# tyler-a-cox/fftvis

Hardware: AMD Instinct MI355X
Metric: simulated visibilities/sec (baselines x freqs x times) at eps=6e-8 (higher is better)
Workload: dtype f64; 1 GPU; C3: hera350, 100000 sources, 128 freqs, 20 times, 61075 baselines, polarized table beam, type3 NUFFT eps=6e-08 upsampfac=2

## Files before the change

### fftvis_amd/csrc/fv_nufft.h

```cpp
#pragma once

#include "fv_eskernel.h"
#include "fv_ydirect.h"

#include <hip/hip_ext.h>

#include <algorithm>
#include <cstdlib>
#include <array>
#include <map>
#include <memory>

namespace fv {

inline bool debug_switch_old_fft() {
    static const bool v = std::getenv("FFTVIS_HIP_OLD_FFT") != nullptr;
    return v;
}
inline bool debug_switch_natural_order() {
    static const bool v = std::getenv("FFTVIS_HIP_NATURAL_ORDER") != nullptr;
    return v;
}

constexpr int BINLOG = 3;
// ... 2701 lines not shown
            DimGeom g;
            g.X = X[d];
            g.B = B[d];
            set_dim_geom(g, sigma, ker.w, scale_max, true, 0.0);
            cells *= g.n2;
        }
        return cells >= 4.0e6 ? -1.0 : 0.0;
    }
    int *col_err = nullptr;
    const unsigned long long *col_omask = nullptr;
    int col_omask_nblk = 0;
    double col_out_cells = 0;
    void arm_columns(const int *tab, const int *xtab, int tpol, int ncc, int *err = nullptr, const unsigned long long *omask = nullptr,
                     int omask_nblk = 0) {
        col_tab = tab && xtab && (dim == 2 || zdirect) && b_block_log() ? tab : nullptr;
        col_xtab = col_tab ? xtab : nullptr;
        col_tab_tpol = tpol;
        col_ncc = ncc;
        col_err = err;
        col_omask = col_tab ? omask : nullptr;
        col_omask_nblk = omask_nblk;
        col_out_cells = 0;
    }
    bool yd_on = false;
    YdArgs yd_args{};
    const int *yd_map = nullptr;
    double yd_cells = 0, yd_pairs = 0;
    DevBuf yd_vals, yd_ones;
    int yd_ones_n = 0;
    const double *yd_scale = nullptr;
    void arm_ydirect(const YdArgs *a, const int *map, double b_cells, const double *scale_dev = nullptr) {
        yd_on = a != nullptr && sizeof(T) == 8 && dim == 2;
        if (!yd_on) return;
        yd_args = *a;
        yd_map = map;
        yd_scale = scale_dev;
        yd_cells = b_cells;
        yd_pairs = (double)a->npts * geo.d[1].na;
    }
    int yd_slots = 0;
    int yd_slot_count() {
        if (!yd_slots) {
            const int smem = (int)yd_smem_bytes();
            int dev = 0, cus = 0, per_cu = 0;
            FV_HIP(hipFuncSetAttribute(reinterpret_cast<const void *>(k_ydirect), hipFuncAttributeMaxDynamicSharedMemorySize, smem));
            FV_HIP(hipOccupancyMaxActiveBlocksPerMultiprocessor(&per_cu, k_ydirect, YD_THREADS, (size_t)smem));
            FV_HIP(hipGetDevice(&dev));
            FV_HIP(hipDeviceGetAttribute(&cus, hipDeviceAttributeMultiprocessorCount, dev));
            yd_slots = std::max(1, per_cu * cus);
        }
        return yd_slots;
    }
    static constexpr int YD_MAX_SLICES = 32;
    void yd_slices(int na_y, int nwg, int nft, int &rps, int &nslices) {
        const int tiles = (int)cdiv(na_y, YD_RT);
        const char *e = std::getenv("FFTVIS_HIP_YD_SLICES");
        int want = e ? std::atoi(e) : 0;
        if (want < 1) {
            const int64_t slots = yd_slot_count(), base = (int64_t)std::max(1, nwg) * std::max(1, nft);
            int64_t best = 0;
            for (int n = 1; n <= std::min(tiles, YD_MAX_SLICES); ++n) {
                const int tps = (int)cdiv(tiles, n), ns = (int)cdiv(tiles, tps);
                const int64_t cost = (2 * cdiv(base * ns, slots) + 1) * (tps + 1);
                if (!want || cost < best) {
                    best = cost;
                    want = n;
                }
            }
        }
        want = std::max(1, std::min(want, tiles));
        rps = (int)cdiv(tiles, want) * YD_RT;
        nslices = (int)cdiv(na_y, rps);
    }
    size_t yd_vals_bytes(int na_y, int nwg, int nfg, int tg, int64_t npts) {
        int rps, ns;
        yd_slices(na_y, nwg, nfg * tg, rps, ns);
        return sizeof(cplx<double>) * (size_t)ns * nfg * tg * (size_t)npts;
    }
    const T *spread_dec_y() {
        if (!yd_on) return dec_cur[1];
        const int n = geo.d[1].na;
        if (yd_ones_n < n) {
            if (yd_ones.p) FV_HIP(hipStreamSynchronize(stream));
            const int cap = std::max(n, 16384);
            yd_ones.reserve(sizeof(double) * (size_t)cap);
            hipLaunchKernelGGL(k_yd_ones, dim3((unsigned)cdiv(cap, 256)), dim3(256), 0, stream, yd_ones.as<double>(), cap);
            yd_ones_n = cap;
        }
        return reinterpret_cast<const T *>(yd_ones.p);
    }
    void ydirect_sum(int ntrans, const cplx<T> *B);
    int ypass_cols_log() const {
        int tpr, rpw;
        rowfft_shape(geo.d[1], true, tpr, rpw);
        return ilog2_c(rpw);
    }
    void build_rowmask(int64_t NU, const T *btx, const T *bty, const int *bl_idx, const signed char *flip, const int *ustart,
                       const double *scale_dev, int nfg, bool both, const int *ctab, int ncc, unsigned long long *mask,
                       int nblk, int nw) const {
        const DimGeom &x = geo.d[0], &y = geo.d[1];
        RowMaskArgs a{};
        a.w = ker.w;
        a.nfg = nfg;
        a.sides = both ? 2 : 1;
        a.n2x = x.n2; a.nox = x.no; a.Px = x.sP(); a.cntx = x.cnt(); a.hx = x.h; a.btcx = x.btc;
        a.n2y = y.n2; a.noy = y.no; a.Py = y.P; a.Qy = y.Q; a.hy = y.h; a.btcy = y.btc;
        a.blk_log = ypass_cols_log();
        a.nblk = nblk;
        a.nw = nw;
        a.ctab_stride = x.nos();
        (void)ncc;
        const int64_t items = NU * nfg * a.sides;
        if (items == 0) return;
        hipLaunchKernelGGL(k_plan_rowmask<T>, dim3((unsigned)cdiv(items, 256)), dim3(256), 0, stream, NU, btx, bty, bl_idx,
                           flip, ustart, scale_dev, a, ctab, mask);
    }
    int xcols() const { return col_tab ? col_ncc : geo.d[0].nos(); }
    int b_block_log_public() const { return b_block_log(); }
    int xcols_with(int ncc) const { return ncc ? ncc : geo.d[0].nos(); }
    int64_t b_pitch_with(int ncc) const { return y_reads_columns() ? (xcols_with(ncc) + 7) / 8 * 8 : xcols_with(ncc); }
    bool columns_possible() const { return (dim == 2 || zdirect) && b_block_log() != 0 && y_reads_columns() && !fused_possible(); }
    bool fused_possible() const;
    bool prepare_fused_gather(int64_t N, const T *btx, const T *bty, const int *bl_idx, const signed char *flip,
                              const double *scale_dev, int nfg, int tpol, cplx<T> *out, int64_t out_fg_stride,
                              int64_t out_k_stride, const int64_t *out_pol_off, int64_t targets_serial = 0,
                              cplx<T> *out_mate = nullptr);
    int64_t M = 0;
    int64_t geom_serial = 0;

// ... 681 lines not shown
    first_pass_ext = row_ext_ptr;
    rowfft(cur, oth, x, tw_cur[0], np, y.na, (int64_t)y.na * x.na, x.na, 1, xp, 0, nullptr, cur1, oth1, 0, blk);
    first_pass_ext = nullptr;
    std::swap(cur, oth);
    std::swap(cur1, oth1);
    if (yd_on) {
        FV_REQUIRE(!mate && !fused_active && dim == 2, "direct y sums: 2-D, stand-alone gather, no gang launch");
        ydirect_sum(ntrans, cur);
        grid_out = cur;
        last_fft_fused = false;
        return;
    }
    if (y_reads_columns()) {
        rowfft(cur, oth, y, tw_cur[1], np, xp, (int64_t)y.na * xp, 1, xp, 0, xcols(),
               fused_active ? &fused_args : nullptr, cur1, oth1, blk, 0);
        std::swap(cur, oth);
        std::swap(cur1, oth1);
    } else {
        dim3 tg((unsigned)cdiv(x.nos(), 32), (unsigned)cdiv(y.na, 32), (unsigned)np);
        hipLaunchKernelGGL(k_transpose<T>, tg, dim3(256), 0, stream, cur, oth, y.na, x.nos());
        if (mate) hipLaunchKernelGGL(k_transpose<T>, tg, dim3(256), 0, stream, cur1, oth1, y.na, x.nos());
        rowfft(oth, cur, y, tw_cur[1], np, x.nos(), (int64_t)x.nos() * y.na, y.na, 1, 0, 0, nullptr,
               oth1, cur1);
    }
    if (dim > 2 && !zdirect) {
        const int64_t nc = (int64_t)x.nos() * y.nos();
        rowfft(cur, oth, z, tw_cur[2], ntrans, nc, (int64_t)z.na * nc, 1, nc);
        std::swap(cur, oth);
    }
    grid_out = cur;
    last_fft_fused = fused_active;
    if (mate) {
        mate->grid_out = cur1;
        mate->last_fft_fused = fused_active;
    }
    fused_active = false;
}

template <typename T>
void Nufft3<T>::ydirect_sum(int ntrans, const cplx<T> *B) {
    if constexpr (sizeof(T) == 8) {
        const DimGeom &y = geo.d[1];
        YdArgs a = yd_args;
        const int tg = ntrans / std::max(1, a.nfg);
        FV_REQUIRE(a.nfg >= 1 && tg * a.nfg == ntrans && (tg == 1 || tg == 2 || tg == 4), "direct y sums: 1, 2 or 4 transforms per frequency");
        const int blk = b_block_log();
        FV_REQUIRE(a.na_y == y.na && a.xp == (int)b_pitch() && a.blk == (blk ? blk : 2) && a.w == ker.w,
                   "direct y sums: the tables were built for another geometry");
        a.plane = (int64_t)y.na * b_pitch();
        a.blk_stride = blk ? ((int64_t)y.na << blk) : 4;
        a.row_stride = blk ? (1 << blk) : b_pitch();
        a.tg = tg;
        FV_REQUIRE(a.blk >= 2 && a.blk <= 4 && a.plane < ((int64_t)1 << 31), "direct y sums: blocks of 4 to 16 elements, 32-bit cell offsets");
        yd_slices(y.na, a.nwg, ntrans, a.rps, a.nslices);
        const size_t need = sizeof(cplx<double>) * (size_t)a.nslices * ntrans * (size_t)a.npts;
        if (yd_vals.cap < need) {
            FV_HIP(hipStreamSynchronize(stream));
            yd_vals.reserve(need);
        }
        yd_args.rps = a.rps;
        yd_args.nslices = a.nslices;
        yd_slot_count();
        const dim3 grid((unsigned)a.nwg, (unsigned)ntrans, (unsigned)a.nslices);
        hipLaunchKernelGGL(k_ydirect, grid, dim3(YD_THREADS), yd_smem_bytes(), stream, reinterpret_cast<const cplx<double> *>(B),
                           yd_scale, a, yd_vals.as<cplx<double>>());
    } else {
        (void)ntrans;
        (void)B;
        FV_REQUIRE(false, "direct y sums: fp64 only");
    }
}

template <typename T>
bool Nufft3<T>::fused_possible() const {
    static const bool off = std::getenv("FFTVIS_HIP_NO_FUSED_GATHER") != nullptr;
    if (off || dim != 2) return false;
    const DimGeom &x = geo.d[0], &y = geo.d[1];
    int tpr, rpw;
    rowfft_shape(y, true, tpr, rpw);
    if (!rowfft_uses_st(y, true) || rpw != 8 || y.logQ > 10) return false;
    if (x.sP() != 1 || y.P != 1) return false;
    const int row_slots = y.logQ == 9 ? 577 : 1153;
    return 2 * y.no <= row_slots && b_pitch() % 8 == 0;
}

template <typename T>
bool Nufft3<T>::prepare_fused_gather(int64_t N, const T *btx, const T *bty, const int *bl_idx,
                                     const signed char *flip, const double *scale_dev, int nfg, int tpol,
                                     cplx<T> *out, int64_t out_fg_stride, int64_t out_k_stride,
                                     const int64_t *out_pol_off, int64_t targets_serial, cplx<T> *out_mate) {
    if (N == 0 || nfg == 0 || tpol > 4 || !fused_possible()) return false;
    const DimGeom &x = geo.d[0], &y = geo.d[1];
    FusedKey key;
    key.serial = geom_serial;
    key.targets = targets_serial;
    key.N = N;
    key.ofs = out_fg_stride;
    key.oks = out_k_stride;
    key.btx = btx;
    key.bl_idx = bl_idx;
    key.flip = flip;
    key.scale = scale_dev;
    key.nfg = nfg;
    key.tpol = tpol;
    const double kg[10] = {x.h, y.h, x.btc, y.btc, x.xc, y.xc, (double)x.no, (double)y.no, (double)x.n2, (double)y.n2};
    for (int i = 0; i < 10; ++i) key.g[i] = kg[i];
    FgGeom gm{};
// ... 240 lines not shown
```

### fftvis_amd/csrc/fv_sim.h

```cpp
#pragma once

#include <atomic>
#include <chrono>
#include <cstdio>
#include <thread>
#include "fv_fit.h"
#include "fv_nufft.h"
#include <unordered_map>

#include <algorithm>
#include <array>
#include <cstdlib>
#include <memory>

namespace fv {

constexpr double SPEED_OF_LIGHT = 299792458.0;

struct BeamDesc {
    int kind;
    int order;
    double diameter;
    double js[8];
    double ps;
// ... 2392 lines not shown
                        hi = std::min(x.no - 1, hi + 1);
                    }
                    for (int i = lo; i <= hi; ++i) row[out_pos(i, P, cnt)] = 1;
                }
            }
            int run = 0;
            for (int i = 0; i < stride; ++i)
                if (row[i]) row[i] = ++run;
            c->ncc = std::max(c->ncc, run);
            if (run * 100 > x.no * 85) c->use = false;
        }
        c->ncc = (c->ncc + 7) / 8 * 8;
        c->yn2 = y.n2; c->yno = y.no; c->yP = y.P; c->yQ = y.Q; c->yh = y.h; c->ybtc = y.btc;
        c->yna = y.na;
        c->blk = n0->b_block_log_public();
        if (c->use) {
            upload(c->tab, tab.data(), sizeof(int) * tab.size(), 0);
            c->h_tab = tab;
            {
                std::vector<int> xt(tab.size());
                const int b = c->blk, rows = y.na << b, mask = (1 << b) - 1;
                for (size_t i = 0; i < tab.size(); ++i) xt[i] = tab[i] ? ((tab[i] - 1) >> b) * rows + ((tab[i] - 1) & mask) + 1 : 0;
                upload(c->xtab, xt.data(), sizeof(int) * xt.size(), 0);
            }
            if (y.logQ >= 9 && y.logQ <= 11 && !std::getenv("FFTVIS_HIP_NO_OUTPUT_MASK")) {
                const int bl = n0->ypass_cols_log(), nw = y.Q > 1024 ? y.Q / 1024 : 1;
                c->nblk = (c->ncc + (1 << bl) - 1) >> bl;
                const size_t words = (size_t)nfg * c->nblk * y.P * nw;
                c->omask.reserve(sizeof(unsigned long long) * words);
                FV_HIP(hipMemsetAsync(c->omask.p, 0, sizeof(unsigned long long) * words, stream));
                hipStream_t keep = n0->stream;
                n0->stream = stream;
                n0->build_rowmask(nu, d_bls.as<T>(), d_bls.as<T>() + nbls, pr.trivial ? nullptr : pr.idx->template as<int>(),
                                  pr.trivial ? nullptr : pr.flip->template as<signed char>(),
                                  pr.ustart ? pr.ustart->template as<int>() : nullptr, d_freqs.as<double>() + fa, nfg, both,
                                  c->tab.template as<int>(), c->ncc, c->omask.template as<unsigned long long>(), c->nblk, nw);
                n0->stream = keep;
                std::vector<unsigned long long> hm(words);
                FV_HIP(hipMemcpyAsync(hm.data(), c->omask.p, sizeof(unsigned long long) * words, hipMemcpyDeviceToHost, stream));
                FV_HIP(hipStreamSynchronize(stream));
                double bits = 0;
                for (unsigned long long v : hm) bits += __builtin_popcountll(v);
                c->out_cells = bits * 16.0 * (1 << bl) / nfg;
            }
        }
        col_plans.push_back(std::move(c));
        return col_plans.back().get();
    }

    struct YPlan {
        int64_t serial;
        int pair, fa, fb;
        const ColPlan *cp;
        int herm, blk, xp, w;
        int xn2, xno, xsP, xcnt, yna, yn2;
        double xh, xbtc, yh, ybtc;
        bool built = false, use = false;
        YdArgs a{};
        double cells = 0;
        DevBuf wg, blkcnt, blkid, cref, xw, ptv, ptg, map;
    };
    std::vector<std::unique_ptr<YPlan>> y_plans;
    std::vector<YPlan *> y_plan_of;
    static double ydirect_gate() { return 1.0; }
    YPlan *ydirect_plan(int pi, const Pair &pr, int fa, int fb, Nufft3<T> *n0, const ColPlan *cp, bool forced) {
        const DimGeom &x = n0->geo.d[0], &y = n0->geo.d[1];
        const int w = n0->ker.w, blkB = n0->b_block_log_public(), blk = blkB ? blkB : 2;
        const int xp = (int)n0->b_pitch_with(cp && cp->use ? cp->ncc : 0);
        for (auto &c : y_plans)
            if (c->serial == targets_serial && c->pair == pi && c->fa == fa && c->fb == fb && c->cp == cp && c->herm == pr.herm &&
                c->blk == (blkB ? blkB : -2) && c->xp == xp && c->w == w && c->xn2 == x.n2 && c->xno == x.no && c->xsP == x.sP() &&
                c->xcnt == x.cnt() && c->yna == y.na && c->yn2 == y.n2 && c->xh == x.h && c->xbtc == x.btc && c->yh == y.h &&
                c->ybtc == y.btc)
                return c.get();
        std::unique_ptr<YPlan> c(new YPlan{targets_serial, pi, fa, fb, cp, pr.herm, blkB ? blkB : -2, xp, w, x.n2, x.no, x.sP(), x.cnt(),
                                           y.na, y.n2, x.h, x.btc, y.h, y.btc});
        y_plans.push_back(std::move(c));
        YPlan *yp = y_plans.back().get();
        const bool dbg = std::getenv("FFTVIS_HIP_DEBUG_YDIRECT") != nullptr;
        auto skip = [&](const char *why) {
            if (dbg) std::fprintf(stderr, "ydirect plan pair %d channels [%d, %d): not built: %s\n", pi, fa, fb, why);
            return yp;
        };
        const int nfg = fb - fa, BE = 1 << blk, sides = pr.herm ? 2 : 1;
        const int64_t N = !pr.h_upairs.empty() ? (int64_t)pr.h_upairs.size() / 2 : !pr.h_ustart.empty() ? (int64_t)pr.h_ustart.size() - 1 : pr.n;
        if (N == 0 || nfg == 0 || w > MAX_W || (pr.herm && (x.btc != 0.0 || y.btc != 0.0))) return skip("no items, or a packed run off centre");
        const size_t NP = (size_t)N * sides;
        std::vector<double> pu(NP), pv(NP);
        for (int64_t i = 0; i < N; ++i) {
            const int64_t ui = !pr.h_upairs.empty() ? pr.h_upairs[2 * i] : i;
            const int64_t kl = pr.h_ustart.empty() ? ui : pr.h_ustart[ui];
            const int64_t k = pr.h_idx[kl];
            const double sg = pr.h_flip[kl] ? -1.0 : 1.0;
            for (int sd = 0; sd < sides; ++sd) {
                const double s2 = sd ? -sg : sg;
                pu[(size_t)i * sides + sd] = s2 * (double)(T)h_bls[k];
                pv[(size_t)i * sides + sd] = s2 * (double)(T)h_bls[(size_t)nbls + k];
            }
        }
        const double tol = std::max(dedup_tol(), 0.0);
        std::vector<int> ord(NP), grp(NP), map(2 * (size_t)N, 0);
        for (size_t i = 0; i < NP; ++i) ord[i] = (int)i;
        std::sort(ord.begin(), ord.end(), [&](int p, int q) { return pu[p] < pu[q] || (pu[p] == pu[q] && (pv[p] < pv[q] || (pv[p] == pv[q] && p < q))); });
        std::vector<double> gu;
        for (size_t i = 0; i < NP; ++i) {
            if (gu.empty() || pu[ord[i]] - gu.back() > tol) gu.push_back(pu[ord[i]]);
            grp[ord[i]] = (int)gu.size() - 1;
        }
        const int G = (int)gu.size();
        std::sort(ord.begin(), ord.end(), [&](int p, int q) { return grp[p] < grp[q] || (grp[p] == grp[q] && (pv[p] < pv[q] || (pv[p] == pv[q] && p < q))); });
        std::vector<double> ptv;
        std::vector<int> ptg, gstart(G + 1, 0);
        for (size_t i = 0; i < NP; ++i) {
            const int q = ord[i];
            if (ptv.empty() || ptg.back() != grp[q] || pv[q] - ptv.back() > tol) {
                ptv.push_back(pv[q]);
                ptg.push_back(grp[q]);
                ++gstart[grp[q] + 1];
            }
            map[(size_t)(q / sides) * 2 + (q % sides)] = (int)ptv.size() - 1;
        }
        for (int g = 0; g < G; ++g) gstart[g + 1] += gstart[g];
        const int64_t npts = (int64_t)ptv.size();
        if (!forced && (double)npts * y.na > ydirect_gate() * ((double)G * w) * 0.5 * y.n2 * std::log2((double)y.n2)) return skip("too many points per u");
        if (blk < 2 || blk > 4) return skip("column blocks of fewer than 4 or more than 16 elements");
        if ((int64_t)y.na * xp >= ((int64_t)1 << 31)) return skip("a plane of B past the kernel's 32-bit cell offsets");
        const int P = x.sP(), cnt = x.cnt(), stride = x.nos(), ncols = n0->xcols_with(cp && cp->use ? cp->ncc : 0);
        const double beta = n0->ker.beta, c4 = n0->ker.c;
        std::vector<int> col((size_t)nfg * G * w);
        std::vector<double> xw((size_t)nfg * G * w);
        for (int fg = 0; fg < nfg; ++fg) {
            const double sc = freqs[fa + fg];
            for (int g = 0; g < G; ++g) {
                const double sv = sc * gu[g], th = x.h * (sv - sc * x.btc);
                const double e = th * x.n2 * (0.5 / M_PI) + 0.5 * x.no;
                const int j = std::max(0, std::min(x.no - w, (int)std::ceil(e - 0.5 * w)));
                for (int q = 0; q < w; ++q) {
                    const int pos = out_pos(std::min(j + q, x.no - 1), P, cnt);
                    int cc = pos;
                    if (cp && cp->use) {
                        const int t = cp->h_tab[(size_t)fg * stride + pos];
                        if (t == 0) return skip("a footprint column the column plan left out");
                        cc = t - 1;
                    }
                    if (cc < 0 || cc >= ncols || cc >= xp) return skip("a column outside B");
                    col[((size_t)fg * G + g) * w + q] = cc;
                    xw[((size_t)fg * G + g) * w + q] = es_eval<double>((double)(j + q) - e, beta, c4);
                }
            }
        }
        const int nbcap = yd_nbcap(blk);
        std::vector<int> wg;
        std::vector<std::vector<int>> cur(nfg), trial(nfg);
        auto blocks_with = [&](int g) {
            int worst = 0;
            for (int fg = 0; fg < nfg; ++fg) {
                trial[fg] = cur[fg];
                for (int q = 0; q < w; ++q) trial[fg].push_back(col[((size_t)fg * G + g) * w + q] >> blk);
                std::sort(trial[fg].begin(), trial[fg].end());
                trial[fg].erase(std::unique(trial[fg].begin(), trial[fg].end()), trial[fg].end());
                worst = std::max(worst, (int)trial[fg].size());
            }
            return worst;
        };
        std::vector<std::vector<int>> range_blocks;
        int g0 = 0;
        while (g0 < G) {
            for (auto &v : cur) v.clear();
            int ng = 0;
            while (g0 + ng < G && ng < YD_NG && gstart[g0 + ng + 1] - gstart[g0] <= YD_THREADS * YD_PTM) {
                if (blocks_with(g0 + ng) > nbcap) break;
                cur.swap(trial);
                ++ng;
            }
            if (ng == 0) return skip("one u-group alone does not fit a workgroup");
            wg.insert(wg.end(), {g0, ng, gstart[g0], gstart[g0 + ng] - gstart[g0]});
            for (int fg = 0; fg < nfg; ++fg) range_blocks.push_back(cur[fg]);
            g0 += ng;
        }
        const int nwg = (int)wg.size() / 4;
        std::vector<int> blkcnt((size_t)nfg * nwg), blkid((size_t)nfg * nwg * YD_NBMAX, 0), cref(col.size());
        double cells = 0;
        for (int r = 0; r < nwg; ++r)
            for (int fg = 0; fg < nfg; ++fg) {
                const std::vector<int> &bl = range_blocks[(size_t)r * nfg + fg];
                blkcnt[(size_t)fg * nwg + r] = (int)bl.size();
                cells += (double)bl.size() * BE * y.na / nfg;
                for (size_t i = 0; i < bl.size(); ++i) blkid[((size_t)fg * nwg + r) * YD_NBMAX + i] = bl[i];
                for (int g = wg[4 * r]; g < wg[4 * r] + wg[4 * r + 1]; ++g)
                    for (int q = 0; q < w; ++q) {
                        const int cc = col[((size_t)fg * G + g) * w + q];
                        const int slot = (int)(std::lower_bound(bl.begin(), bl.end(), cc >> blk) - bl.begin());
                        cref[((size_t)fg * G + g) * w + q] = (slot << 4) | (cc & (BE - 1));
                    }
            }
        upload(yp->wg, wg.data(), sizeof(int) * wg.size(), 0);
        upload(yp->blkcnt, blkcnt.data(), sizeof(int) * blkcnt.size(), 0);
        upload(yp->blkid, blkid.data(), sizeof(int) * blkid.size(), 0);
        upload(yp->cref, cref.data(), sizeof(int) * cref.size(), 0);
        upload(yp->xw, xw.data(), sizeof(double) * xw.size(), 0);
        upload(yp->ptv, ptv.data(), sizeof(double) * ptv.size(), 0);
        upload(yp->ptg, ptg.data(), sizeof(int) * ptg.size(), 0);
        upload(yp->map, map.data(), sizeof(int) * map.size(), 0);
        YdArgs &a = yp->a;
        a.w = w;
        a.nfg = nfg;
        a.nwg = nwg;
        a.ngroups = G;
        a.na_y = y.na;
        a.xp = xp;
        a.blk = blk;
        a.npts = npts;
        a.hy = y.h;
        a.btcy = y.btc;
        a.wg = yp->wg.template as<int>();
        a.blkcnt = yp->blkcnt.template as<int>();
        a.blkid = yp->blkid.template as<int>();
        a.cref = yp->cref.template as<int>();
        a.xw = yp->xw.template as<double>();
        a.ptv = yp->ptv.template as<double>();
        a.ptg = yp->ptg.template as<int>();
        yp->cells = cells;
        yp->built = true;
        std::vector<int> dc(col.begin() + (size_t)(nfg - 1) * G * w, col.end());
        std::sort(dc.begin(), dc.end());
        const double columns = (double)(std::unique(dc.begin(), dc.end()) - dc.begin());
        const double direct = (double)npts * y.na, ypass = columns * 0.5 * y.n2 * std::log2((double)y.n2);
        yp->use = n0->columns_possible() && n0->geo.cells_o() >= 4000000 && direct <= ydirect_gate() * ypass;
        if (dbg)
            std::fprintf(stderr, "ydirect plan pair %d channels [%d, %d): %lld items, %lld points on %d u-groups, %d work ranges, %.0f columns, "
                         "B cells read %.3g of %.3g needed, na_y %d, blocks of %d, plan %d, rule %.2f -> %s\n", pi, fa, fb, (long long)N,
                         (long long)npts, G, nwg, columns, cells, columns * y.na, y.na, BE, cp ? 1 : 0, direct / ypass, yp->use ? "taken" : "not taken");
        return yp;
    }

    void set_basis(int nant, int K, int nfreq, const void *coefs, const int *ant1,
                   const int *ant2) override {
        FV_HIP(hipSetDevice(device));
        FV_REQUIRE(polarized, "basis beams need a polarized engine (wrapper.py:280-283)");
        FV_REQUIRE(nbls > 0 && K >= 1 && K == (int)beams.size(), "set_array and the K basis beams first");
        FV_REQUIRE(nfreq == (int)freqs.size(), "beam_coefs frequency axis != freqs");
        for (int64_t b = 0; b < nbls; ++b)
            FV_REQUIRE(ant1[b] >= 0 && ant1[b] < nant && ant2[b] >= 0 && ant2[b] < nant, "antenna index out of range");
        nbasis = K;
        nant_basis = nant;
        {
            std::vector<int> start(nant + 1, 0), list((size_t)2 * nbls);
            for (int64_t b = 0; b < nbls; ++b) {
                ++start[ant1[b] + 1];
                ++start[ant2[b] + 1];
            }
            for (int a = 0; a < nant; ++a) start[a + 1] += start[a];
            std::vector<int> fill(start.begin(), start.end() - 1);
            for (int64_t b = 0; b < nbls; ++b) {
                list[fill[ant1[b]]++] = (int)(2 * b);
                list[fill[ant2[b]]++] = (int)(2 * b + 1);
            }
            upload(d_csr_start, start.data(), sizeof(int) * start.size(), 0);
            upload(d_csr, list.data(), sizeof(int) * list.size(), 0);
        }
        upload(d_coefs, coefs, sizeof(cplx<T>) * (size_t)nant * K * nfreq, 0);
        upload(d_ant1, ant1, sizeof(int) * nbls, 0);
        upload(d_ant2, ant2, sizeof(int) * nbls, 0);
        std::vector<int> bi, bj, idx(nbls);
        std::vector<int64_t> off(1, 0);
        std::vector<int> all;
        std::vector<signed char> fl;
        for (int k = 0; k < K; ++k)
            for (int l = k; l < K; ++l) {
                bi.push_back(k);
                bj.push_back(l);
                for (int64_t b = 0; b < nbls; ++b) {
                    all.push_back((int)b);
                    fl.push_back(0);
                }
                off.push_back((int64_t)all.size());
            }
        set_beam_pairs((int)bi.size(), bi.data(), bj.data(), off.data(), all.data(), fl.data());
    }

    void set_chunking(int nchunks, double sb) override {
        FV_REQUIRE(nchunks >= 1, "nchunks must be >= 1");
        FV_REQUIRE(sb > 0.0 && sb <= 1.0, "source_buffer must be in (0, 1]");
        src_chunks = nchunks;
        source_buffer = sb;
// ... 893 lines not shown
        }
        for (auto &cpo : col_plan_of) cpo.assign(r.groups.size() * pairs.size(), nullptr);
        if (col_plans.size() > 512) {
            FV_HIP(hipDeviceSynchronize());
            col_plans.clear();
            y_plans.clear();
        }
        if (y_plans.size() > 512) {
            FV_HIP(hipDeviceSynchronize());
            y_plans.clear();
        }
        y_plan_of.assign(r.groups.size() * pairs.size(), nullptr);
        for (int c = 0; c < r.ncls; ++c) {
            if (std::getenv("FFTVIS_HIP_NO_COLUMN_PLAN")) break;
            Nufft3<T> *n0 = lanes[0].plan[c].get();
            if (n0->dim != 2 && !n0->zdirect) continue;
            for (size_t gi = 0; gi < r.groups.size(); ++gi) {
                const double smax = fmax_of(r.groups[gi].first, r.groups[gi].second);
                for (size_t pi = 0; pi < pairs.size(); ++pi) {
                    const Pair &pr = pairs[pi];
                    if (pr.n == 0) continue;
                    n0->grid_slack = 0.0;
                    n0->set_geometry(r.xc, r.X, pr.box_c(), pr.box_B(), smax);
                    if (!n0->columns_possible() || n0->geo.cells_o() < 4000000) continue;
                    col_plan_of[c][gi * pairs.size() + pi] = column_plan((int)pi, pr, r.groups[gi].first, r.groups[gi].second, n0);
                }
            }
            FV_HIP(hipStreamSynchronize(n0->stream));
        }
        const char *ey = std::getenv("FFTVIS_HIP_YDIRECT");
        const int ymode = ey ? std::atoi(ey) : -1;
        if (!r.forward || ymode == 0 || sizeof(T) != 8 || r.D != 2 || r.gang || nbasis || r.K || r.nsets()) return;
        Nufft3<T> *n0 = lanes[0].plan[0].get();
        size_t vals_need = 0;
        for (size_t gi = 0; gi < r.groups.size(); ++gi) {
            const int fa = r.groups[gi].first, fb = r.groups[gi].second;
            const double smax = fmax_of(fa, fb);
            for (size_t pi = 0; pi < pairs.size(); ++pi) {
                const Pair &pr = pairs[pi];
                const int tg = pr.herm ? 2 : tpol;
                if (pr.n == 0 || tg > 4 || pr.mirror) continue;
                const ColPlan *cp = col_plan_of[0][gi * pairs.size() + pi];
                if (cp && !cp->use) cp = nullptr;
                n0->grid_slack = cp ? 0.0 : -1.0;
                n0->set_geometry(r.xc, r.X, pr.box_c(), pr.box_B(), smax);
                if (ymode != 1 && (!n0->columns_possible() || n0->geo.cells_o() < 4000000)) continue;
                if (n0->fused_possible() && ymode != 1) continue;
                YPlan *yp = ydirect_plan((int)pi, pr, fa, fb, n0, cp, ymode == 1);
                if (!yp->built || !(ymode == 1 || yp->use)) continue;
                y_plan_of[gi * pairs.size() + pi] = yp;
                vals_need = std::max(vals_need, n0->yd_vals_bytes(yp->a.na_y, yp->a.nwg, fb - fa, tg, yp->a.npts));
                if (std::getenv("FFTVIS_HIP_DEBUG_YDIRECT")) {
                    int rps, ns;
                    n0->yd_slices(yp->a.na_y, yp->a.nwg, (fb - fa) * tg, rps, ns);
                    const int wgs = yp->a.nwg * (fb - fa) * tg * ns;
                    std::fprintf(stderr, "ydirect launch pair %d channels [%d, %d): %d slices of %d rows (na_y %d), %d workgroups, %d per round\n",
                                 (int)pi, fa, fb, ns, rps, yp->a.na_y, wgs, n0->yd_slot_count());
                }
            }
        }
        FV_HIP(hipStreamSynchronize(n0->stream));
        if (vals_need)
            for (int li = 0; li < r.nlanes_used; ++li) {
                lanes[li].plan[0]->yd_vals.reserve(vals_need);
                lanes[li].plan[0]->yd_slots = n0->yd_slots;
            }
    }

    void queue_units(const RunPlan &r, const OutBlock &o, Drain &dr, cplx<double> *const *gs = nullptr) {
        const int t0 = r.t0, t1 = r.t1, f0 = r.f0, nt = r.nt, D = r.D, nch = r.ch.n;
        const int64_t csz = r.ch.csz, cap = r.ch.cap;
        const bool pipe = r.pipe, gang = r.gang;
        const auto &groups = r.groups;
        const int64_t per_tf = o.per_tf;
        const std::array<int64_t, 16> pol_off = pol_offsets();
        if (r.nlanes > 1 && !pipe) {
            FV_HIP(hipEventRecord(ev_start, stream));
            for (int li = 1; li < r.nlanes; ++li) FV_HIP(hipStreamWaitEvent(lanes[li].stream, ev_start, 0));
        }

        const int sample_step = std::min(TIMING_STRIDE / 2, nt - 1);
        const Pair *last_pair = nullptr;
        for (const Pair &pr : pairs)
            if (pr.n) last_pair = &pr;
        int active_pairs = 0;
        for (const Pair &pr : pairs) active_pairs += pr.n > 0;
        const char *erh = std::getenv("FFTVIS_HIP_RIDE_EVENT");
        const bool ride_heavy_done = !(erh && std::atoi(erh) == 0) && groups.size() == 1 && active_pairs == 1;
        for (int tnext = t0, ch = 0; tnext < t1;) {
            const int nm = gang && tnext + 1 < t1 ? 2 : 1;
            const int tu = tnext;
            const int64_t s0 = (int64_t)ch * csz, sn = std::min<int64_t>(csz, nsrc - s0);
            const bool accumulate = ch > 0;
            const int chunk = ch;
            if (++ch == nch) {
                ch = 0;
                tnext += nm;
            }
            hipStream_t unit_stream = stream;
            auto close_time = [&]() {
                if (!o.drain || chunk != nch - 1) return;
                const hipEvent_t ev = drain_event(dr.items.size());
                FV_HIP(hipEventRecord(ev, unit_stream));
                dr.items.push_back({ev, tu - t0, nm});
                if (dr.pin.pinned()) drain_flush(o, dr);
            };
            if (nsrc == 0 || sn <= 0) {
// ... 1437 lines not shown
```

### fftvis_amd/csrc/fv_ydirect.h

```cpp
#pragma once

#include "fv_eskernel.h"

namespace fv {

constexpr int YD_THREADS = 512;
constexpr int YD_RT = 32;
constexpr int YD_NG = 8;
constexpr int YD_PTM = 2;
constexpr int YD_NBMAX = 20;
constexpr int YD_RAWROW = 100;
constexpr int YD_RAW = YD_RAWROW * YD_RT;
constexpr int YD_NLD = 5;
constexpr int YD_RESEED = 128;
constexpr int YD_WCH = 4;
constexpr int YD_RCH = 4;
static_assert(2 * YD_NG * YD_RT == YD_THREADS, "one contraction item per pair of threads");
static_assert(YD_RESEED % YD_RT == 0, "seeds fall on tile starts");
static_assert(YD_RT == 32 && YD_RT % YD_RCH == 0, "a tile row index is five bits (k_ydirect's shifts)");
static_assert(MAX_W % YD_WCH == 0, "whole chunks of footprint cells");

__host__ __device__ constexpr int yd_nbcap(int blk) {
    const int a = YD_RAWROW / ((1 << blk) + 1), b = (YD_NLD * YD_THREADS / YD_RT) >> blk;
    return a < b ? (a < YD_NBMAX ? a : YD_NBMAX) : (b < YD_NBMAX ? b : YD_NBMAX);
}

struct YdArgs {
    int w, nfg, nwg, ngroups;
    int na_y, xp;
    int blk;
    int64_t blk_stride, row_stride;
    int rps, nslices;
    int tg;
    int64_t plane;
    int64_t npts;
    double hy, btcy;
    const int *wg;
    const int *blkcnt;
    const int *blkid;
    const int *cref;
    const double *xw;
    const double *ptv;
    const int *ptg;
};

inline size_t yd_smem_bytes() {
    return sizeof(cplx<double>) * (size_t)(YD_RAW + YD_NG * YD_RT) + sizeof(double) * YD_NG * MAX_W +
           sizeof(int) * (YD_NG * MAX_W + YD_NBMAX);
}

__global__ __launch_bounds__(YD_THREADS, 4) void k_ydirect(const cplx<double> *__restrict__ B, const double *__restrict__ scale,
                                                          YdArgs a, cplx<double> *__restrict__ vals) {
    extern __shared__ __attribute__((aligned(16))) unsigned char yd_smem[];
    cplx<double> *raw = reinterpret_cast<cplx<double> *>(yd_smem);
    cplx<double> *D = raw + YD_RAW;
    double *xw_s = reinterpret_cast<double *>(D + YD_NG * YD_RT);
    int *cref_s = reinterpret_cast<int *>(xw_s + YD_NG * MAX_W);
    int *bid_s = cref_s + YD_NG * MAX_W;
    const int tid = threadIdx.x, wgi = blockIdx.x, ft = blockIdx.y, fg = ft / a.tg, sl = blockIdx.z;
    const int g0 = a.wg[4 * wgi], ng = min(a.wg[4 * wgi + 1], YD_NG), p0 = a.wg[4 * wgi + 2],
              np = min(a.wg[4 * wgi + 3], YD_THREADS * YD_PTM);
    const int BE = 1 << a.blk, BEP = BE + 1;
    const int nb = min(a.blkcnt[fg * a.nwg + wgi], yd_nbcap(a.blk));
    const int rbeg = sl * a.rps, rend = min(a.na_y, rbeg + a.rps);
    for (int i = tid; i < ng * a.w; i += YD_THREADS) {
        const int gi = i / a.w, g = i - gi * a.w;
        const int64_t src = ((int64_t)fg * a.ngroups + g0 + gi) * a.w + g;
        const int c = a.cref[src];
        xw_s[gi * MAX_W + g] = a.xw[src];
        cref_s[gi * MAX_W + g] = (min(c >> 4, nb - 1) * YD_RT * BEP + (c & (BE - 1))) * (int)sizeof(cplx<double>);
    }
    if (tid < nb) bid_s[tid] = a.blkid[((int64_t)fg * a.nwg + wgi) * YD_NBMAX + tid];
    const double sc = scale[fg];
    double th[YD_PTM], dr[YD_PTM], di[YD_PTM], er[YD_PTM], ei[YD_PTM], accr[YD_PTM], acci[YD_PTM];
    int dofs[YD_PTM];
    bool kon[YD_PTM];
#pragma unroll
    for (int k = 0; k < YD_PTM; ++k) {
        const int p = tid + k * YD_THREADS;
        kon[k] = k * YD_THREADS + (tid & ~63) < np;
        const int gp = p0 + (p < np ? p : 0);
        th[k] = a.hy * (sc * a.ptv[gp] - sc * a.btcy);
        dofs[k] = min(max(a.ptg[gp] - g0, 0), YD_NG - 1) * YD_RT;
        sincos(th[k], &di[k], &dr[k]);
        er[k] = 1.0;
        ei[k] = 0.0;
        accr[k] = acci[k] = 0.0;
    }
    const int citem = tid >> 1, cpart = tid & 1;
    const int cgi = citem / YD_RT, crow = citem % YD_RT;
    const int half = a.na_y / 2;
    const int per = YD_RT << a.blk, pshift = a.blk + 5;
    __syncthreads();
    const int lrow = (tid & (per - 1)) >> a.blk, lel = tid & (BE - 1), lbstep = YD_THREADS >> pshift;
    const int lofs = ((tid >> pshift) * YD_RT + lrow) * BEP + lel, lstep = lbstep * YD_RT * BEP;
    unsigned goff[YD_NLD], live = 0;
#pragma unroll
    for (int j = 0; j < YD_NLD; ++j) {
        const int lb = (tid >> pshift) + j * lbstep;
        goff[j] = 0;
        if (lb < nb) {
            const int bid = bid_s[lb];
            if ((bid << a.blk) + lel < a.xp) {
                goff[j] = (unsigned)((int64_t)bid * a.blk_stride + (int64_t)lrow * a.row_stride + lel);
                live |= 1u << j;
            }
        }
    }
    const cplx<double> *plane = B + (int64_t)ft * a.plane;
    cplx<double> pf[YD_NLD];
    for (int r0 = rbeg - YD_RT; r0 < rend; r0 += YD_RT) {
        if (r0 >= rbeg) {
            const unsigned ok = r0 + lrow < rend ? live : 0;
#pragma unroll
            for (int j = 0; j < YD_NLD; ++j) raw[lofs + j * lstep] = (ok >> j) & 1 ? pf[j] : cplx<double>{0.0, 0.0};
        }
        if (r0 + YD_RT < rend) {
            const cplx<double> *base = plane + (int64_t)(r0 + YD_RT) * a.row_stride;
            const bool rowin = r0 + YD_RT + lrow < rend;
#pragma unroll
            for (int j = 0; j < YD_NLD; ++j) pf[j] = base[rowin ? goff[j] : 0u];
        }
        if (r0 < rbeg) continue;
        __syncthreads();
        if (cgi < ng) {
            const char *mine = reinterpret_cast<const char *>(raw) + (crow * BEP * 2 + cpart) * (int)sizeof(double);
            double sum = 0.0;
            for (int gb = 0; gb < a.w; gb += YD_WCH) {
                int c[YD_WCH];
                double wv[YD_WCH], v[YD_WCH];
#pragma unroll
                for (int q = 0; q < YD_WCH; ++q) {
                    c[q] = cref_s[cgi * MAX_W + gb + q];
                    wv[q] = xw_s[cgi * MAX_W + gb + q];
                }
#pragma unroll
                for (int q = 0; q < YD_WCH; ++q)
                    v[q] = *reinterpret_cast<const double *>(mine + (gb + q < a.w ? c[q] : 0));
#pragma unroll
                for (int q = 0; q < YD_WCH; ++q)
                    if (gb + q < a.w) sum += v[q] * wv[q];
            }
            reinterpret_cast<double *>(D)[2 * (cgi * YD_RT + crow) + cpart] = sum;
        }
        __syncthreads();
        if ((r0 - rbeg) % YD_RESEED == 0) {
#pragma unroll
            for (int k = 0; k < YD_PTM; ++k)
                if (kon[k]) sincos(th[k] * (double)(r0 - half), &ei[k], &er[k]);
        }
#pragma unroll
        for (int k = 0; k < YD_PTM; ++k) {
            if (!kon[k]) continue;
            const cplx<double> *d = D + dofs[k];
#pragma unroll 1
            for (int rb = 0; rb < YD_RT; rb += YD_RCH) {
                cplx<double> v[YD_RCH];
#pragma unroll
                for (int q = 0; q < YD_RCH; ++q) v[q] = d[rb + q];
#pragma unroll
                for (int q = 0; q < YD_RCH; ++q) {
                    accr[k] += v[q].re * er[k] - v[q].im * ei[k];
                    acci[k] += v[q].re * ei[k] + v[q].im * er[k];
                    const double e2 = er[k] * dr[k] - ei[k] * di[k];
                    ei[k] = er[k] * di[k] + ei[k] * dr[k];
                    er[k] = e2;
                }
            }
        }
    }
#pragma unroll
    for (int k = 0; k < YD_PTM; ++k) {
        const int p = tid + k * YD_THREADS;
        if (p < np) vals[((int64_t)sl * a.nfg * a.tg + ft) * a.npts + p0 + p] = {accr[k], acci[k]};
    }
}

__global__ void k_yd_ones(double *__restrict__ tab, int n) {
    const int i = blockIdx.x * blockDim.x + threadIdx.x;
    if (i < n) tab[i] = 1.0;
}

}
```

Baseline: 215.4 million visibilities/s.

## Pair opposite-sign y targets in direct sums and hoist carrier rotation

Groups targets within each u-group whose y coordinates are near negatives of each other, so one walk slot evaluates both sums. It keeps four partial products instead of two accumulators and recombines them into the +y and -y outputs through a slot-to-point map. The common carrier phase (the btc offset) is moved out of the per-target phase and applied once per row, on the column sums, with a rotating factor held in shared memory. The slice-count cost model also gains a term for output gather volume. The aim is to roughly halve the per-target inner-loop work, at the cost of extra shared memory, a tolerance-based pairing that may alter accuracy, and a modified slice heuristic.

After: 234.9 million visibilities/s, median of 6. 1.09x the previous value.

```diff
diff --git a/fftvis_amd/csrc/fv_nufft.h b/fftvis_amd/csrc/fv_nufft.h
--- a/fftvis_amd/csrc/fv_nufft.h
+++ b/fftvis_amd/csrc/fv_nufft.h
@@ -2777,7 +2777,8 @@
         return yd_slots;
     }
     static constexpr int YD_MAX_SLICES = 32;
-    void yd_slices(int na_y, int nwg, int nft, int &rps, int &nslices) {
+    static constexpr int64_t YD_GATHER_VALUES_PER_UNIT = 72000;
+    void yd_slices(int na_y, int nwg, int nft, int64_t npts, int &rps, int &nslices) {
         const int tiles = (int)cdiv(na_y, YD_RT);
         const char *e = std::getenv("FFTVIS_HIP_YD_SLICES");
         int want = e ? std::atoi(e) : 0;
@@ -2786,7 +2787,8 @@
             int64_t best = 0;
             for (int n = 1; n <= std::min(tiles, YD_MAX_SLICES); ++n) {
                 const int tps = (int)cdiv(tiles, n), ns = (int)cdiv(tiles, tps);
-                const int64_t cost = (2 * cdiv(base * ns, slots) + 1) * (tps + 1);
+                const int64_t cost = (2 * cdiv(base * ns, slots) + 1) * (tps + 1)
+                                     + (int64_t)ns * std::max(1, nft) * std::max<int64_t>(npts, 0) / YD_GATHER_VALUES_PER_UNIT;
                 if (!want || cost < best) {
                     best = cost;
                     want = n;
@@ -2799,7 +2801,7 @@
     }
     size_t yd_vals_bytes(int na_y, int nwg, int nfg, int tg, int64_t npts) {
         int rps, ns;
-        yd_slices(na_y, nwg, nfg * tg, rps, ns);
+        yd_slices(na_y, nwg, nfg * tg, npts, rps, ns);
         return sizeof(cplx<double>) * (size_t)ns * nfg * tg * (size_t)npts;
     }
     const T *spread_dec_y() {
@@ -3587,7 +3589,7 @@
         a.row_stride = blk ? (1 << blk) : b_pitch();
         a.tg = tg;
         FV_REQUIRE(a.blk >= 2 && a.blk <= 4 && a.plane < ((int64_t)1 << 31), "direct y sums: blocks of 4 to 16 elements, 32-bit cell offsets");
-        yd_slices(y.na, a.nwg, ntrans, a.rps, a.nslices);
+        yd_slices(y.na, a.nwg, ntrans, a.npts, a.rps, a.nslices);
         const size_t need = sizeof(cplx<double>) * (size_t)a.nslices * ntrans * (size_t)a.npts;
         if (yd_vals.cap < need) {
             FV_HIP(hipStreamSynchronize(stream));
diff --git a/fftvis_amd/csrc/fv_sim.h b/fftvis_amd/csrc/fv_sim.h
--- a/fftvis_amd/csrc/fv_sim.h
+++ b/fftvis_amd/csrc/fv_sim.h
@@ -2468,13 +2468,13 @@
         int64_t serial;
         int pair, fa, fb;
         const ColPlan *cp;
-        int herm, blk, xp, w;
+        int herm, blk, xp, w, pairing;
         int xn2, xno, xsP, xcnt, yna, yn2;
         double xh, xbtc, yh, ybtc;
         bool built = false, use = false;
         YdArgs a{};
         double cells = 0;
-        DevBuf wg, blkcnt, blkid, cref, xw, ptv, ptg, map;
+        DevBuf wg, blkcnt, blkid, cref, xw, slv, slg, slp, map;
     };
     std::vector<std::unique_ptr<YPlan>> y_plans;
     std::vector<YPlan *> y_plan_of;
@@ -2483,13 +2483,15 @@
         const DimGeom &x = n0->geo.d[0], &y = n0->geo.d[1];
         const int w = n0->ker.w, blkB = n0->b_block_log_public(), blk = blkB ? blkB : 2;
         const int xp = (int)n0->b_pitch_with(cp && cp->use ? cp->ncc : 0);
+        const char *epair = std::getenv("FFTVIS_HIP_YD_PAIRS");
+        const int pairing = epair && std::atoi(epair) == 0 ? 0 : 1;
         for (auto &c : y_plans)
             if (c->serial == targets_serial && c->pair == pi && c->fa == fa && c->fb == fb && c->cp == cp && c->herm == pr.herm &&
-                c->blk == (blkB ? blkB : -2) && c->xp == xp && c->w == w && c->xn2 == x.n2 && c->xno == x.no && c->xsP == x.sP() &&
+                c->blk == (blkB ? blkB : -2) && c->xp == xp && c->w == w && c->pairing == pairing && c->xn2 == x.n2 && c->xno == x.no && c->xsP == x.sP() &&
                 c->xcnt == x.cnt() && c->yna == y.na && c->yn2 == y.n2 && c->xh == x.h && c->xbtc == x.btc && c->yh == y.h &&
                 c->ybtc == y.btc)
                 return c.get();
-        std::unique_ptr<YPlan> c(new YPlan{targets_serial, pi, fa, fb, cp, pr.herm, blkB ? blkB : -2, xp, w, x.n2, x.no, x.sP(), x.cnt(),
+        std::unique_ptr<YPlan> c(new YPlan{targets_serial, pi, fa, fb, cp, pr.herm, blkB ? blkB : -2, xp, w, pairing, x.n2, x.no, x.sP(), x.cnt(),
                                            y.na, y.n2, x.h, x.btc, y.h, y.btc});
         y_plans.push_back(std::move(c));
         YPlan *yp = y_plans.back().get();
@@ -2580,6 +2582,9 @@
             return worst;
         };
         std::vector<std::vector<int>> range_blocks;
+        std::vector<double> slv;
+        std::vector<int> slg, slp;
+        int64_t npairs = 0;
         int g0 = 0;
         while (g0 < G) {
             for (auto &v : cur) v.clear();
@@ -2590,7 +2595,29 @@
                 ++ng;
             }
             if (ng == 0) return skip("one u-group alone does not fit a workgroup");
-            wg.insert(wg.end(), {g0, ng, gstart[g0], gstart[g0 + ng] - gstart[g0]});
+            const int s0 = (int)slv.size();
+            for (int g = g0; g < g0 + ng; ++g) {
+                auto single = [&](int p) {
+                    slv.push_back(ptv[p]);
+                    slg.push_back(g);
+                    slp.insert(slp.end(), {p, -1});
+                };
+                int lo = gstart[g], hi = gstart[g + 1] - 1;
+                while (lo <= hi) {
+                    const double sum = ptv[lo] + ptv[hi];
+                    if (pairing && lo < hi && ptv[lo] < 0.0 && ptv[hi] > 0.0 && std::fabs(sum) <= tol) {
+                        slv.push_back(ptv[hi]);
+                        slg.push_back(g);
+                        slp.insert(slp.end(), {hi--, lo++});
+                        ++npairs;
+                    } else if (pairing && lo < hi && sum > 0.0) {
+                        single(hi--);
+                    } else {
+                        single(lo++);
+                    }
+                }
+            }
+            wg.insert(wg.end(), {g0, ng, s0, (int)slv.size() - s0});
             for (int fg = 0; fg < nfg; ++fg) range_blocks.push_back(cur[fg]);
             g0 += ng;
         }
@@ -2615,8 +2642,9 @@
         upload(yp->blkid, blkid.data(), sizeof(int) * blkid.size(), 0);
         upload(yp->cref, cref.data(), sizeof(int) * cref.size(), 0);
         upload(yp->xw, xw.data(), sizeof(double) * xw.size(), 0);
-        upload(yp->ptv, ptv.data(), sizeof(double) * ptv.size(), 0);
-        upload(yp->ptg, ptg.data(), sizeof(int) * ptg.size(), 0);
+        upload(yp->slv, slv.data(), sizeof(double) * slv.size(), 0);
+        upload(yp->slg, slg.data(), sizeof(int) * slg.size(), 0);
+        upload(yp->slp, slp.data(), sizeof(int) * slp.size(), 0);
         upload(yp->map, map.data(), sizeof(int) * map.size(), 0);
         YdArgs &a = yp->a;
         a.w = w;
@@ -2634,8 +2662,9 @@
         a.blkid = yp->blkid.template as<int>();
         a.cref = yp->cref.template as<int>();
         a.xw = yp->xw.template as<double>();
-        a.ptv = yp->ptv.template as<double>();
-        a.ptg = yp->ptg.template as<int>();
+        a.slv = yp->slv.template as<double>();
+        a.slg = yp->slg.template as<int>();
+        a.slp = yp->slp.template as<int>();
         yp->cells = cells;
         yp->built = true;
         std::vector<int> dc(col.begin() + (size_t)(nfg - 1) * G * w, col.end());
@@ -2647,6 +2676,9 @@
             std::fprintf(stderr, "ydirect plan pair %d channels [%d, %d): %lld items, %lld points on %d u-groups, %d work ranges, %.0f columns, "
                          "B cells read %.3g of %.3g needed, na_y %d, blocks of %d, plan %d, rule %.2f -> %s\n", pi, fa, fb, (long long)N,
                          (long long)npts, G, nwg, columns, cells, columns * y.na, y.na, BE, cp ? 1 : 0, direct / ypass, yp->use ? "taken" : "not taken");
+        if (dbg)
+            std::fprintf(stderr, "ydirect slots pair %d channels [%d, %d): %lld pairs, %lld singles, %lld walk slots for %lld points\n", pi, fa, fb,
+                         (long long)npairs, (long long)(npts - 2 * npairs), (long long)slv.size(), (long long)npts);
         return yp;
     }
 
@@ -3646,7 +3678,7 @@
                 vals_need = std::max(vals_need, n0->yd_vals_bytes(yp->a.na_y, yp->a.nwg, fb - fa, tg, yp->a.npts));
                 if (std::getenv("FFTVIS_HIP_DEBUG_YDIRECT")) {
                     int rps, ns;
-                    n0->yd_slices(yp->a.na_y, yp->a.nwg, (fb - fa) * tg, rps, ns);
+                    n0->yd_slices(yp->a.na_y, yp->a.nwg, (fb - fa) * tg, yp->a.npts, rps, ns);
                     const int wgs = yp->a.nwg * (fb - fa) * tg * ns;
                     std::fprintf(stderr, "ydirect launch pair %d channels [%d, %d): %d slices of %d rows (na_y %d), %d workgroups, %d per round\n",
                                  (int)pi, fa, fb, ns, rps, yp->a.na_y, wgs, n0->yd_slot_count());
diff --git a/fftvis_amd/csrc/fv_ydirect.h b/fftvis_amd/csrc/fv_ydirect.h
--- a/fftvis_amd/csrc/fv_ydirect.h
+++ b/fftvis_amd/csrc/fv_ydirect.h
@@ -19,6 +19,7 @@
 static_assert(YD_RESEED % YD_RT == 0, "seeds fall on tile starts");
 static_assert(YD_RT == 32 && YD_RT % YD_RCH == 0, "a tile row index is five bits (k_ydirect's shifts)");
 static_assert(MAX_W % YD_WCH == 0, "whole chunks of footprint cells");
+static_assert(YD_PTM <= 4 && YD_NG * YD_RT / YD_RCH <= 256, "a byte per slot holds its place in D (k_ydirect's dofs)");
 
 __host__ __device__ constexpr int yd_nbcap(int blk) {
     const int a = YD_RAWROW / ((1 << blk) + 1), b = (YD_NLD * YD_THREADS / YD_RT) >> blk;
@@ -40,12 +41,13 @@
     const int *blkid;
     const int *cref;
     const double *xw;
-    const double *ptv;
-    const int *ptg;
+    const double *slv;
+    const int *slg;
+    const int *slp;
 };
 
 inline size_t yd_smem_bytes() {
-    return sizeof(cplx<double>) * (size_t)(YD_RAW + YD_NG * YD_RT) + sizeof(double) * YD_NG * MAX_W +
+    return sizeof(cplx<double>) * (size_t)(YD_RAW + YD_NG * YD_RT + YD_THREADS + 1) + sizeof(double) * (YD_NG * MAX_W + YD_PTM * YD_THREADS) +
            sizeof(int) * (YD_NG * MAX_W + YD_NBMAX);
 }
 
@@ -54,8 +56,10 @@
     extern __shared__ __attribute__((aligned(16))) unsigned char yd_smem[];
     cplx<double> *raw = reinterpret_cast<cplx<double> *>(yd_smem);
     cplx<double> *D = raw + YD_RAW;
-    double *xw_s = reinterpret_cast<double *>(D + YD_NG * YD_RT);
-    int *cref_s = reinterpret_cast<int *>(xw_s + YD_NG * MAX_W);
+    cplx<double> *rot_s = D + YD_NG * YD_RT;
+    double *xw_s = reinterpret_cast<double *>(rot_s + YD_THREADS + 1);
+    double *th_s = xw_s + YD_NG * MAX_W;
+    int *cref_s = reinterpret_cast<int *>(th_s + YD_PTM * YD_THREADS);
     int *bid_s = cref_s + YD_NG * MAX_W;
     const int tid = threadIdx.x, wgi = blockIdx.x, ft = blockIdx.y, fg = ft / a.tg, sl = blockIdx.z;
     const int g0 = a.wg[4 * wgi], ng = min(a.wg[4 * wgi + 1], YD_NG), p0 = a.wg[4 * wgi + 2],
@@ -72,23 +76,34 @@
     }
     if (tid < nb) bid_s[tid] = a.blkid[((int64_t)fg * a.nwg + wgi) * YD_NBMAX + tid];
     const double sc = scale[fg];
-    double th[YD_PTM], dr[YD_PTM], di[YD_PTM], er[YD_PTM], ei[YD_PTM], accr[YD_PTM], acci[YD_PTM];
-    int dofs[YD_PTM];
+    const double beta = a.hy * (sc * a.btcy);
+    if (beta != 0.0) {
+        cplx<double> f;
+        sincos(beta * (double)(sl * a.rps + (tid >> 1) % YD_RT - a.na_y / 2), &f.im, &f.re);
+        rot_s[tid] = f;
+        if (tid == 0) {
+            sincos(beta * (double)YD_RT, &f.im, &f.re);
+            rot_s[YD_THREADS] = f;
+        }
+    }
+    double dr[YD_PTM], di[YD_PTM], er[YD_PTM], ei[YD_PTM], sp[YD_PTM], sq[YD_PTM], sr[YD_PTM], ss[YD_PTM];
+    unsigned dofs = 0;
     bool kon[YD_PTM];
 #pragma unroll
     for (int k = 0; k < YD_PTM; ++k) {
         const int p = tid + k * YD_THREADS;
         kon[k] = k * YD_THREADS + (tid & ~63) < np;
         const int gp = p0 + (p < np ? p : 0);
-        th[k] = a.hy * (sc * a.ptv[gp] - sc * a.btcy);
-        dofs[k] = min(max(a.ptg[gp] - g0, 0), YD_NG - 1) * YD_RT;
-        sincos(th[k], &di[k], &dr[k]);
+        const double th = a.hy * (sc * a.slv[gp]);
+        th_s[p] = th;
+        dofs |= (unsigned)(min(max(a.slg[gp] - g0, 0), YD_NG - 1) * (YD_RT / YD_RCH)) << (8 * k);
+        sincos(th, &di[k], &dr[k]);
         er[k] = 1.0;
         ei[k] = 0.0;
-        accr[k] = acci[k] = 0.0;
+        sp[k] = sq[k] = sr[k] = ss[k] = 0.0;
     }
     const int citem = tid >> 1, cpart = tid & 1;
-    const int cgi = citem / YD_RT, crow = citem % YD_RT;
+    const int cgi = __builtin_amdgcn_readfirstlane(citem / YD_RT), crow = citem % YD_RT;
     const int half = a.na_y / 2;
     const int per = YD_RT << a.blk, pshift = a.blk + 5;
     __syncthreads();
@@ -141,18 +156,24 @@
                 for (int q = 0; q < YD_WCH; ++q)
                     if (gb + q < a.w) sum += v[q] * wv[q];
             }
+            if (beta != 0.0) {
+                const cplx<double> f = rot_s[tid], st = rot_s[YD_THREADS];
+                const double other = __shfl_xor(sum, 1);
+                sum = cpart ? sum * f.re - other * f.im : sum * f.re + other * f.im;
+                rot_s[tid] = {f.re * st.re - f.im * st.im, f.re * st.im + f.im * st.re};
+            }
             reinterpret_cast<double *>(D)[2 * (cgi * YD_RT + crow) + cpart] = sum;
         }
         __syncthreads();
         if ((r0 - rbeg) % YD_RESEED == 0) {
 #pragma unroll
             for (int k = 0; k < YD_PTM; ++k)
-                if (kon[k]) sincos(th[k] * (double)(r0 - half), &ei[k], &er[k]);
+                if (kon[k]) sincos(th_s[tid + k * YD_THREADS] * (double)(r0 - half), &ei[k], &er[k]);
         }
 #pragma unroll
         for (int k = 0; k < YD_PTM; ++k) {
             if (!kon[k]) continue;
-            const cplx<double> *d = D + dofs[k];
+            const cplx<double> *d = D + ((dofs >> (8 * k)) & 255u) * YD_RCH;
 #pragma unroll 1
             for (int rb = 0; rb < YD_RT; rb += YD_RCH) {
                 cplx<double> v[YD_RCH];
@@ -160,8 +181,10 @@
                 for (int q = 0; q < YD_RCH; ++q) v[q] = d[rb + q];
 #pragma unroll
                 for (int q = 0; q < YD_RCH; ++q) {
-                    accr[k] += v[q].re * er[k] - v[q].im * ei[k];
-                    acci[k] += v[q].re * ei[k] + v[q].im * er[k];
+                    sp[k] += v[q].re * er[k];
+                    sq[k] += v[q].im * ei[k];
+                    sr[k] += v[q].re * ei[k];
+                    ss[k] += v[q].im * er[k];
                     const double e2 = er[k] * dr[k] - ei[k] * di[k];
                     ei[k] = er[k] * di[k] + ei[k] * dr[k];
                     er[k] = e2;
@@ -172,7 +195,11 @@
 #pragma unroll
     for (int k = 0; k < YD_PTM; ++k) {
         const int p = tid + k * YD_THREADS;
-        if (p < np) vals[((int64_t)sl * a.nfg * a.tg + ft) * a.npts + p0 + p] = {accr[k], acci[k]};
+        if (p >= np) continue;
+        cplx<double> *out = vals + ((int64_t)sl * a.nfg * a.tg + ft) * a.npts;
+        const int pp = a.slp[2 * (p0 + p)], pm = a.slp[2 * (p0 + p) + 1];
+        if (pp >= 0 && pp < a.npts) out[pp] = {sp[k] - sq[k], sr[k] + ss[k]};
+        if (pm >= 0 && pm < a.npts) out[pm] = {sp[k] + sq[k], ss[k] - sr[k]};
     }
 }
 
```
